# 123456jack/decision-making-and-path-planning

Measured on NVIDIA B200. Metric: trajectories_scored_per_s, higher is better.
Workload: dtype f64

## Files before the change

### decision-making-and-path-planning_b200/csrc/dp_cycle.cu

```cuda
#include <cstdlib>
#include "dp_device.cuh"
#include "dp_fused.cuh"
#include "dp_kernels.h"
#include "dp_group.cuh"

namespace {

struct Beh { int behavior, target, light; bool lanechg, obsavoid; int dlg; };

struct Slice { int base, stride, P; double d; };

__device__ __forceinline__ void put_slot(dp_search_slot* slot, const SearchRes& r, int evaluated, int lane) {
    if (slot && lane == 0) {
        slot->dis_lat = r.dis_lat; slot->dis_lng = r.dis_lng; slot->ob_index = (int16_t)r.ob;
        slot->pathid = (uint16_t)r.pathid; slot->evaluated = (uint8_t)evaluated; slot->found = r.found ? 1 : 0;
        slot->pad[0] = slot->pad[1] = 0;
    }
}

__device__ __forceinline__ void lane_slices(const DevMap& m, int gl, int id, int id_more, Slice& fwd, Slice& rear, int& ub) {
    const int off = m.lane_pt_off[gl], n = m.lane_pt_off[gl + 1] - off;
    const int a = min(n, id + id_more), b = min(n, id + 120 + id_more);
    fwd.base = off + a; fwd.stride = 1; fwd.P = max(0, b - a); fwd.d = 0.0;
    const int lo = max(0, id + id_more - 40);
// ... 32 lines not shown
                sm.scr[j] = m.lenp[off + i0 + j];
            }
            const unsigned bad = __ballot_sync(DP_FULL, !ok);
            if (bad) { first_bad = j0 + __ffs(bad) - 1; break; }
        }
        const int cn = min(cnt, first_bad);
        __syncwarp();
        dp_pad_scr(sm, cn, lane);
        __syncwarp();
        const SeqHit hq = dp_seq_first(sm, cn, sum, 0.0, thr);
        if (hq.k >= 0) return true;
        sum = hq.acc;
        if (first_bad < cnt) break;
    }
    return sum > thr;
}

static __device__ __noinline__ int aim_walk_lane(const DevMap& m, WarpSmem& sm, int gl_walk, int from, int to_excl, float faraim, int lane) {
    if (from >= to_excl) return -2;
    const int off = m.lane_pt_off[gl_walk], n = m.lane_pt_off[gl_walk + 1] - off;
    if (from < 0) return -3;
    if (to_excl > n - 1) { to_excl = n - 1; if (from >= to_excl) return -3; }
    double sum = 0.0;
    for (int i0 = from; i0 < to_excl; i0 += DP_SCR) {
        const int cnt = min(DP_SCR, to_excl - i0);
        __syncwarp();
        for (int j = lane; j < cnt; j += 32) sm.scr[j] = m.lenp[off + i0 + j];
        dp_pad_scr(sm, cnt, lane);
        __syncwarp();
        const SeqHit hq = dp_seq_first(sm, cnt, sum, 4.0, (double)faraim);
        if (hq.k >= 0) return i0 + hq.k;
        sum = hq.acc;
    }
    return -1;
}

__device__ __forceinline__ Src junction_src(const DevMap& m, int base0, int n0, int base1, int n1) {
    Src s = dp_src_run(m.xy + base0, 1, n0);
    s.p1 = m.xy + base1; s.n1 = n1;
    return s;
}

__device__ __forceinline__ void junction_recipe(const DevMap& m, const dp_scene_hdr& h, int& base0, int& n0, int& base1, int& n1) {
    const int gc = (h.conn >= 0 && h.conn < m.n_conn) ? m.conn[h.conn].lane : -1;
    const int coff = gc >= 0 ? m.lane_pt_off[gc] : 0, n_inter = gc >= 0 ? m.lane_pt_off[gc + 1] - coff : 0;
    const int gj = m.road_lane_base[h.road_num - 1] + h.lane_num - 1;
    const int off = m.lane_pt_off[gj], n = m.lane_pt_off[gj + 1] - off;
    if (h.pos == 1) {
        const int idj = (int)(uint16_t)h.id[h.lane_num - 1];
        base0 = off + idj; n0 = max(0, n - idj);
        base1 = coff; n1 = n_inter;
    } else {
        const int idj = (int)(uint16_t)h.id[h.last_lanenum - 1];
        base0 = coff + idj; n0 = max(0, n_inter - idj);
        base1 = off; n1 = min(60, n);
    }
}

static __device__ __noinline__ SearchRes dp_search_cold(const Src s, double mx, double my, const double* ox, const double* oy, int N,
                                                        const LaneMap lm, double lo, double hi, WarpSmem& sm, int lane, float hb = 0.f,
                                                        float dmax = 0.f) {
    return dp_search(s, mx, my, ox, oy, N, lm, lo, hi, sm, lane, hb, dmax);
}

__device__ __forceinline__ void dp_publish(unsigned* flag, unsigned epoch, int lane) {
    __syncwarp();
    if (lane == 0) asm volatile("st.release.gpu.global.u32 [%0], %1;" ::"l"(flag), "r"(epoch) : "memory");
}
__device__ __forceinline__ void dp_await(const unsigned* flag, unsigned epoch) {
    unsigned v = 0;
#pragma unroll 1
    for (int spin = 0; spin < (1 << 22); ++spin) {
        asm volatile("ld.acquire.gpu.global.u32 %0, [%1];" : "=r"(v) : "l"(flag) : "memory");
        if (v == epoch) break;
        __nanosleep(spin < 64 ? 100 : 1000);
    }
    if (v != epoch) __trap();
    __syncwarp();
}
template <class T> __device__ __forceinline__ T dp_l2(const T* p) { return __ldcg(p); }

}

#ifndef DP_PRUNE_REGION
#define DP_PRUNE_REGION 0
#endif
#ifndef DP_PRUNE_LOCAL
#define DP_PRUNE_LOCAL 0
#endif
#ifndef DP_PRUNE_SWEEP
#define DP_PRUNE_SWEEP (WPB == 4)
#endif
#define DP_CARVEOUT 77
#ifndef DP_MIN_BLOCKS_W1
#define DP_MIN_BLOCKS_W1 25
#endif
#define DP_MIN_BLOCKS(WPB) ((WPB) == 1 ? DP_MIN_BLOCKS_W1 : 7)

#ifdef DP_DEBUG_CLOCK
__device__ long long g_dbg_timeline[2 * 65536 * 2 * 8];
__device__ __forceinline__ long long dbg_now() { unsigned long long t; asm volatile("mov.u64 %0, %globaltimer;" : "=l"(t)); return (long long)t; }
#define DBG_MARK(ph, slot) if (lane == 0) g_dbg_timeline[(((size_t)(io.epoch & 1) * 65536 + scene) * 2 + (ph)) * 8 + (slot)] = dbg_now()
#define DBG_END(ph, nt) if (lane == 0) { long long* g = g_dbg_timeline + (((size_t)(io.epoch & 1) * 65536 + scene) * 2 + (ph)) * 8; g[1] = dbg_now(); g[3] = (nt); }
extern "C" int dp_debug_scene_timeline(long long* dst, int n_scenes) {
    (void)n_scenes;
    return (int)cudaMemcpyFromSymbol(dst, g_dbg_timeline, sizeof(g_dbg_timeline));
}
#else
#define DBG_MARK(ph, slot)
#define DBG_END(ph, nt)
#endif

template <int PHASE, int WPB>
__global__ void __launch_bounds__(WPB * 32, DP_MIN_BLOCKS(WPB))
dp_cycle_kernel(DevMap m, dp_params p, int n_scenes, const dp_scene_hdr* __restrict__ hdr, const double* __restrict__ obs_x,
                const double* __restrict__ obs_y, int max_obs, dp_carry* __restrict__ carry, double2* __restrict__ last_path,
                dp_plan_record* __restrict__ rec, dp_trace_record* __restrict__ trace, double* __restrict__ path_xy,
                double* __restrict__ path_ll, DpIo io) {
    __shared__ WarpSmem smem[WPB];
    const int lane = threadIdx.x & 31, wib = threadIdx.x >> 5;
    const int scene = blockIdx.x * WPB + wib;
    if (scene >= n_scenes) return;
#ifdef DP_DEBUG_CLOCK
    if (lane == 0) {
        unsigned sid;
        asm volatile("mov.u32 %0, %smid;" : "=r"(sid));
        long long* g = g_dbg_timeline + (((size_t)(io.epoch & 1) * 65536 + scene) * 2 + (PHASE == 2 ? 1 : 0)) * 8;
        g[0] = dbg_now(); g[2] = sid; g[4] = g[5] = g[6] = 0;
    }
    const long long dbg_t0 = clock64();
    long long dbg_t[8] = {0, 0, 0, 0, 0, 0, 0, 0};
#define DBG_T(i) dbg_t[i] = clock64() - dbg_t0
#else
#define DBG_T(i)
#endif
    WarpSmem& sm = smem[wib];
    if (PHASE == 1 && io.done) asm volatile("griddepcontrol.launch_dependents;" ::: "memory");
    if (PHASE == 2 && io.pdone) asm volatile("griddepcontrol.launch_dependents;" ::: "memory");
    if (PHASE == 1 && io.in_flag) dp_await(io.in_flag, io.epoch);
    if (PHASE == 2 && io.done) dp_await(io.done + scene, io.epoch);
    if (PHASE == 1 && !io.in_flag && !io.hdr_stage && lane < 5) {
        const size_t row = (size_t)scene * max_obs, last = (size_t)(max_obs > 0 ? max_obs - 1 : 0);
        const void* a = lane == 0 ? (const void*)(obs_x + row) : lane == 1 ? (const void*)(obs_x + row + last)
                      : lane == 2 ? (const void*)(obs_y + row) : lane == 3 ? (const void*)(obs_y + row + last) : (const void*)(carry + scene);
        asm volatile("prefetch.global.L2 [%0];" ::"l"(a));
    }
    sm.hdr[lane] = (PHASE == 2 || io.in_flag) ? dp_l2(reinterpret_cast<const uint32_t*>(hdr + scene) + lane)
                                              : reinterpret_cast<const uint32_t*>(hdr + scene)[lane];
    __syncwarp();
    const dp_scene_hdr& h = *reinterpret_cast<const dp_scene_hdr*>(sm.hdr);
    const double* ox = obs_x + (size_t)scene * max_obs;
    const double* oy = obs_y + (size_t)scene * max_obs;
    const int N = min((int)h.n_obs, max_obs);
    if (PHASE != 2 && io.hdr_stage) {
        reinterpret_cast<uint32_t*>(io.hdr_stage + scene)[lane] = sm.hdr[lane];
        for (int k = lane; k < N; k += 32) {
            io.ox_stage[(size_t)scene * max_obs + k] = ox[k];
            io.oy_stage[(size_t)scene * max_obs + k] = oy[k];
        }
    }
    double2* lastp = last_path + (size_t)scene * DP_PATH_POINTS;
    dp_carry* const cg = carry + scene;
    dp_plan_record* const out = rec + scene;
    if (PHASE == 1 && io.prev_epoch) dp_await(io.pdone + scene, io.prev_epoch);
    uint32_t fwd_w = 0;
    if (PHASE != 2 && io.n_fwd) fwd_w = __ldcg(reinterpret_cast<const uint32_t*>(io.fwd_src + scene) + lane);
    const LaneMap lm = dp_lane_map(N, lane);
    const bool lm_act = (lm.nchunk > 1) && (lane < N * lm.nchunk);
    const bool via_l2 = PHASE == 2 || io.in_flag != nullptr;
    const double mx = lm_act ? (via_l2 ? dp_l2(ox + lm.o) : ox[lm.o]) : 0.0, my = lm_act ? (via_l2 ? dp_l2(oy + lm.o) : oy[lm.o]) : 0.0;
    dp_trace_record* tr = trace ? trace + scene : nullptr;
    if (tr && PHASE != 2) {
        uint32_t* w = reinterpret_cast<uint32_t*>(tr);
        for (int i = lane; i < (int)(sizeof(dp_trace_record) / 4); i += 32) w[i] = 0;
        __syncwarp();
    }
    const double Vw = p.vehicle_width;
    const int pos = h.pos;
    int ub = 0, n_traj = 0, pts = 0;
    int rp_base0 = 0, rp_n0 = 0, rp_base1 = 0, rp_n1 = 0;
    int gl = 0, lane_sum = 0;
    const int lane_n = h.lane_num;
    int d_behavior = 1, d_target = 0;
    double v_exp = 10.0;

    if (PHASE == 2) {
        d_behavior = dp_l2(&cg->behavior); d_target = dp_l2(&cg->target_lanenum); v_exp = dp_l2(&cg->velocity_expect);
        n_traj = dp_l2(&out->n_traj);
        if (tr) { ub = dp_l2(&tr->ub_hits); pts = (int)dp_l2(&tr->pts_scored); }
        if (pos == 0) {
            gl = m.road_lane_base[h.road_num - 1] + lane_n - 1;
            lane_sum = m.road_lane_base[h.road_num] - m.road_lane_base[h.road_num - 1];
        } else if (pos == 1 || pos == 2) junction_recipe(m, h, rp_base0, rp_n0, rp_base1, rp_n1);
    } else if (pos == 0) {
        const int road = h.road_num;
        gl = m.road_lane_base[road - 1] + lane_n - 1;
        lane_sum = m.road_lane_base[road] - m.road_lane_base[road - 1];
        const int off = m.lane_pt_off[gl], id_sum = m.lane_pt_off[gl + 1] - off;
        const int id = (int)(uint16_t)h.id[lane_n - 1];
        unsigned navi = 4, navi_t = 0;
        for (int i = 0; i < DP_LANESUM && h.out_lane_no[i] != 0; ++i)
            if (lane_n == h.out_lane_no[i]) { navi = 0; break; }
        int out_min = h.out_lane_no[0], out_max = 1;
        for (int i = 0; i < DP_LANESUM; ++i) if (h.out_lane_no[i] > out_max) out_max = h.out_lane_no[i];
        if (navi == 4) {
            int dirn = 0;
            if (lane_n < out_min) { navi = 2; dirn = 2; }
            else if (lane_n > out_max) { navi = 1; dirn = 1; }
            else navi = 0;
            if (dirn) {
                int times = 5;
                for (int i = 0; i < DP_LANESUM && h.out_lane_no[i] != 0; ++i) {
                    const int t = (dirn == 1) ? lane_n - h.out_lane_no[i] : h.out_lane_no[i] - lane_n;
                    if (t < times) times = t;
                }
                navi_t = (unsigned)(times & 0xff);
            }
        }
        const int idc = min(id, id_sum - 1);
        const int lanechg = m.attr[off + idc];
        const double W = m.width[off + idc] / 100.0;
        Slice F, R, NF, NR;
        NF.base = NR.base = 0; NF.stride = 1; NR.stride = -1; NF.P = NR.P = 0; NF.d = NR.d = 0.0;
        lane_slices(m, gl, id, p.id_more, F, R, ub);
        int side = 0, gn = gl;
        if (lanechg == 1 || lanechg == 3) {
            side = 1;
            if (lane_n > 1) {
                const int idl = (int)(uint16_t)h.id[lane_n - 2];
                const int nl = m.lane_pt_off[gl] - m.lane_pt_off[gl - 1];
                if (idl > 0 && idl < nl) { lane_slices(m, gl - 1, idl, p.id_more, NF, NR, ub); gn = gl - 1; }
            } else { NF = F; NF.d = -1 * W; NR = R; NR.d = -1 * W; }
        } else if (lanechg == 2) {
            side = 2;
            if (lane_n < lane_sum) {
                const int idr = (int)(uint16_t)h.id[lane_n];
                const int nr = m.lane_pt_off[gl + 2] - m.lane_pt_off[gl + 1];
                if (idr > 0 && idr < nr) { lane_slices(m, gl + 1, idr, p.id_more, NF, NR, ub); gn = gl + 1; }
            } else { NF = F; NF.d = W; NR = R; NR.d = W; }
        }
        const int nslot = (side == 2) ? 4 : 2;
        double gF = 0.0, gNF = 0.0, gNR = 0.0;
        double bdF = 0.0;
        {
            const int rb[4] = {F.base, R.base, NF.base, NR.base}, rs[4] = {F.stride, R.stride, NF.stride, NR.stride};
            const int rP[4] = {F.P, R.P, NF.P, NR.P};
            const double rd[4] = {0.0, 0.0, NF.d, NR.d};
            dp_region_stage(m, sm, rb, rs, rP, rd, lane);
            const double nlo = (side == 2) ? -0.5 * W : -0.5 * Vw, nhi = (side == 2) ? 0.5 * Vw : 0.5 * W;
            float hbF, dmF, hbN, dmN;
            dg_bounds(m, gl, 0.0, -0.5 * Vw, 0.5 * Vw, &hbF, &dmF);
            dg_bounds(m, gn, NF.d, nlo, nhi, &hbN, &dmN);
            int qoff = 0;
            bdF = __longlong_as_double(0x7ff0000000000000LL);
#pragma unroll 1
            for (int r = 0; r < 4; ++r) {
                const int Pr = (r == 0) ? F.P : (r == 1) ? R.P : (r == 2) ? NF.P : NR.P;
                if (Pr != 0) {
                    Src sp = dp_src_run(m.xy, 1, Pr);
                    sp.q_off = qoff;
                    const SearchRes sr = dp_search(sp, mx, my, ox, oy, N, lm, r < 2 ? -0.5 * Vw : nlo, r < 2 ? 0.5 * Vw : nhi, sm, lane,
                                                   DP_PRUNE_REGION ? (r < 2 ? hbF : hbN) : 0.f, r < 2 ? dmF : dmN, r == 0 ? &bdF : nullptr);
                    ++n_traj; pts += Pr;
                    put_slot(tr ? &tr->region[r < 2 ? r : nslot + r - 2] : nullptr, sr, 1, lane);
                    if (r == 0) gF = sr.dis_lng; else if (r == 2) gNF = sr.dis_lng; else if (r == 3) gNR = sr.dis_lng;
                }
                qoff += Pr;
            }
        }
        const double gLF = (side == 1) ? gNF : 0.0, gLR = (side == 1) ? gNR : 0.0;
        const double gRF = (side == 2) ? gNF : 0.0, gRR = (side == 2) ? gNR : 0.0;
        if (tr && lane == 0) { tr->width_curlane = W; tr->navi_lanechg = navi; tr->navi_lanechg_times = navi_t; }
        DBG_T(5);
        DBG_MARK(0, 4);

        dp_carry c;
        if (PHASE == 1) {
            const int4* src = reinterpret_cast<const int4*>(cg);
            int4* dst = reinterpret_cast<int4*>(&c);
#pragma unroll
            for (int k = 0; k < (int)(sizeof(dp_carry) / 16); ++k) dst[k] = __ldcg(src + k);
        } else c = *cg;
        Beh cur;
        cur.behavior = c.behavior; cur.target = c.target_lanenum; cur.light = c.light_status;
        cur.lanechg = c.lanechg_status != 0; cur.obsavoid = c.obsavoid_status != 0; cur.dlg = c.behavior_to_dlg;
        const int his_behavior = c.his_behavior, his_target = c.his_target_lanenum, his_light = c.his_light_status;
        int lane_cur = lane_n;
        int z_light = c.light_status;
        int sweep_pick = -1;
        const double period = h.period_ms;
        int K = 0;
        while (K < DP_MAX_SWEEP && (double)K < (W - Vw) / 0.6) ++K;
#define DP_KEEP(reset) do { cur.behavior = 1; cur.target = lane_cur; if (reset) cur.lanechg = false; } while (0)
#define DP_TICK do { c.leftlight_time += period; if (c.leftlight_time > 2000) c.leftlight_time = 2000; } while (0)
        if (lanechg == 0) {
            if (gF < 15) {
                c.no_obsavoid_time = 0;
                c.obsavoid_time++;
                if (c.obsavoid_time > 2) {
                    const int total = 2 * K, shifted = 2 * (K - 1);
                    DBG_MARK(0, 5);
                    if (shifted > 0 && N > 0 && N <= 16) {
                        dp_sweep_stage(m, sm, F.base, F.P, lane);
                        const float hmaxF = m.lane_hmax[gl], hminF = m.lane_hmin[gl], dnF = m.lane_dnmax[gl];
                        unsigned relmask = (N >= 32) ? 0xffffffffu : ((1u << N) - 1u);
                        {
                            const float adm = 0.3f * (float)(K - 1) * 1.0001f;
                            const float hbm = hmaxF + adm * dnF + 1e-4f;
                            const float dlt = (hminF > 1e-6f) ? dnF * (1.0f + 4.0f * adm / hminF) * 1.0001f + 1e-6f : 2.0f;
                            const float dmm = dg_dmax(-0.5 * Vw, 0.5 * Vw, hbm, dlt, hminF - adm * dnF);
                            const bool rel = lane < N && !(sqrt(bdF) - (double)adm > (double)dmm * 1.000001 + 1e-6);
                            relmask &= __ballot_sync(DP_FULL, rel);
                            if (relmask == 0u) relmask = 1u;
                        }
                        const int M = __popc(relmask);
                        const int per = min(8, 32 / M);
                        const int oid = (int)__fns(relmask, 0, lane % M + 1);
                        const double smx = __shfl_sync(DP_FULL, mx, oid), smy = __shfl_sync(DP_FULL, my, oid);
                        for (int u0 = 0; u0 < shifted && (sweep_pick < 0 || tr); u0 += per) {
                            const int cnt = min(per, shifted - u0);
                            const bool none_yet = sweep_pick < 0;
                            int first_g = -1;
                            const int first = dp_sweep_pass(sm, F.P, u0, cnt, K, smx, smy, M, lm, -0.5 * Vw, 0.5 * Vw, 25.0, tr != nullptr, lane,
                                [&](int g, const SearchRes& r, bool before_first) {
                                    if (before_first && r.dis_lng > 25) first_g = g;
                                    if (tr) put_slot(&tr->sweep[(g / K) * DP_MAX_SWEEP + (g % K)], r, (none_yet && before_first) ? 1 : 2, lane);
                                }, DP_PRUNE_SWEEP ? hmaxF : -1.f, hminF, dnF, oid, relmask);
                            if (sweep_pick < 0 && first >= 0) sweep_pick = first_g;
                        }
                    } else {
                        for (int u = 0; u < shifted && (sweep_pick < 0 || tr); ++u) {
                            const int g = dp_sweep_g(u, K);
                            const double cd = dp_sweep_offset(g, K);
                            float hbC, dmC;
                            dg_bounds(m, gl, cd, -0.5 * Vw, 0.5 * Vw, &hbC, &dmC);
                            const SearchRes s = dp_search_cold(slice_src(m, F.base, 1, F.P, cd), mx, my, ox, oy, N, lm, -0.5 * Vw, 0.5 * Vw, sm, lane, hbC, dmC);
                            const bool before = sweep_pick < 0;
                            put_slot(tr ? &tr->sweep[(g / K) * DP_MAX_SWEEP + (g % K)] : nullptr, s, before ? 1 : 2, lane);
                            if (before && s.dis_lng > 25) sweep_pick = g;
                        }
                    }
                    {
                        const int scored = sweep_pick < 0 ? total : sweep_pick + 1;
                        n_traj += scored; pts += scored * F.P;
                        if (tr && total > 0) {
                            __syncwarp();
                            if (lane == 0) {
                                dp_search_slot s0 = tr->region[0];
                                s0.evaluated = 1; tr->sweep[0] = s0;
                                s0.evaluated = (uint8_t)(K < scored ? 1 : 2); tr->sweep[DP_MAX_SWEEP] = s0;
                            }
// ... 741 lines not shown
```

### decision-making-and-path-planning_b200/csrc/dp_device.cuh

```cuda
#pragma once
#include <cuda_runtime.h>
#include <stdint.h>
#include "../../include/dmpp_b200.h"
#include "dp_group.cuh"

#define DP_FULL 0xffffffffu
#define DP_TILE 120
#define DP_SCR 192
#ifndef DP_WARPS_PER_BLOCK
#define DP_WARPS_PER_BLOCK 4
#endif

typedef DgMap DevMap;

struct __align__(16) WarpSmem {
    union {
        struct {
            double2 plan[DP_PATH_POINTS];
            double2 tile[DP_TILE];
        };
        double2 q[DP_PATH_POINTS + DP_TILE];
    };
    double scr[DP_SCR + 8];
    unsigned long long mbar;
    unsigned long long pad_;
    uint32_t hdr[32];
};

struct Src {
    const double2* p0; int stride0; int n0;
    const double2* p1; int n1;
    const double2* nrm0;
    double d;
    int q_off;
};
struct LaneMap { int nchunk, o, c; unsigned magic; };
__device__ __forceinline__ int dp_div_chunks(int x, const LaneMap& lm) { return (int)(((unsigned)x * lm.magic) >> 20); }
struct SearchRes { bool found; double dis_lat, dis_lng; int ob, pathid; };

__device__ __forceinline__ LaneMap dp_lane_map(int N, int lane) {
    LaneMap lm;
    if (N >= 32 || N <= 0) { lm.nchunk = 1; lm.o = lane; lm.c = 0; }
    else { lm.nchunk = 32 / N; lm.c = lane / N; lm.o = lane - lm.c * N; }
    lm.magic = (1u << 20) / (unsigned)lm.nchunk + 1u;
    return lm;
}
__device__ __forceinline__ double dp_sq2(double dx, double dy) { return fma(dx, dx, dy * dy); }
__device__ __forceinline__ double dp_dist_plain(double ax, double ay, double bx, double by) {
    double dx = ax - bx, dy = ay - by;
    return sqrt(dx * dx + dy * dy);
}
__device__ __forceinline__ double2 dp_normal(double2 a, double2 b) {
    double sx = b.x - a.x, sy = b.y - a.y;
    double len = sqrt(dp_sq2(sx, sy));
    if (len > 0) return make_double2(sy / len, -sx / len);
    return make_double2(0.0, 0.0);
}
__device__ __forceinline__ Src dp_src_run(const double2* p, int stride, int n) {
    Src s;
    s.p0 = p; s.stride0 = stride; s.n0 = n; s.p1 = p; s.n1 = 0; s.nrm0 = nullptr; s.d = 0.0; s.q_off = -1;
    return s;
}
__device__ __forceinline__ double2 dp_src_point(const Src& s, int j) {
    if (j >= s.n0) return s.p1[j - s.n0];
    double2 q = s.p0[s.stride0 * j];
    if (s.d != 0.0 && s.n0 >= 2) {
        const int jj = min(j, s.n0 - 2);
        double2 n = (s.stride0 > 0) ? s.nrm0[jj] : s.nrm0[-jj - 1];
        if (s.stride0 < 0) { n.x = -n.x; n.y = -n.y; }
        q.x = fma(s.d, n.x, q.x); q.y = fma(s.d, n.y, q.y);
    }
    return q;
}

__device__ __forceinline__ void dp_pad_scr(WarpSmem& sm, int n, int lane) {
    if (lane < 8) sm.scr[n + lane] = 0.0;
}
__device__ __forceinline__ double dp_seq_sum(const WarpSmem& sm, int n, double acc) {
#pragma unroll 1
    for (int j = 0; j < n; j += 8) {
        const double t0 = sm.scr[j], t1 = sm.scr[j + 1], t2 = sm.scr[j + 2], t3 = sm.scr[j + 3];
        const double t4 = sm.scr[j + 4], t5 = sm.scr[j + 5], t6 = sm.scr[j + 6], t7 = sm.scr[j + 7];
        acc += t0; acc += t1; acc += t2; acc += t3; acc += t4; acc += t5; acc += t6; acc += t7;
    }
    return acc;
}
struct SeqHit { int k; double acc; };
__device__ __forceinline__ SeqHit dp_seq_first(const WarpSmem& sm, int n, double acc, double sub, double thr) {
    SeqHit r;
#pragma unroll 1
    for (int j = 0; j < n; j += 8) {
        const double t0 = sm.scr[j], t1 = sm.scr[j + 1], t2 = sm.scr[j + 2], t3 = sm.scr[j + 3];
        const double t4 = sm.scr[j + 4], t5 = sm.scr[j + 5], t6 = sm.scr[j + 6], t7 = sm.scr[j + 7];
        const double s0 = acc + t0, s1 = s0 + t1, s2 = s1 + t2, s3 = s2 + t3, s4 = s3 + t4, s5 = s4 + t5, s6 = s5 + t6, s7 = s6 + t7;
        if ((s7 - sub) > thr) {
            int k = j + 7;
            if ((s6 - sub) > thr) k = j + 6;
            if ((s5 - sub) > thr) k = j + 5;
            if ((s4 - sub) > thr) k = j + 4;
            if ((s3 - sub) > thr) k = j + 3;
            if ((s2 - sub) > thr) k = j + 2;
            if ((s1 - sub) > thr) k = j + 1;
            if ((s0 - sub) > thr) k = j;
            if (k < n) { r.k = k; r.acc = acc; return r; }
        }
        acc = s7;
    }
    r.k = -1; r.acc = acc;
    return r;
}

__device__ __forceinline__ int dp_nearest_plain(const double2* pts, int n, double x, double y, int lane) {
    const double INF = __longlong_as_double(0x7ff0000000000000LL), TOL = 1.0 + 0x1p-49;
    double be = INF;
    int bi = 0x7fffffff;
    bool amb = false;
    for (int i = lane; i < n; i += 32) {
        const double2 q = pts[i];
        const double dx = x - q.x, dy = y - q.y;
        const double e = dx * dx + dy * dy;
        if (e < be) { amb = amb || (be <= e * TOL); be = e; bi = i; }
    }
    double ge = be;
    int gi = bi;
#pragma unroll
    for (int o = 16; o > 0; o >>= 1) {
        const double oe = __shfl_xor_sync(DP_FULL, ge, o);
        const int oi = __shfl_xor_sync(DP_FULL, gi, o);
        if (oe < ge || (oe == ge && oi < gi)) { ge = oe; gi = oi; }
    }
    amb = amb || (be != ge && be <= ge * TOL);
    if (!__any_sync(DP_FULL, amb)) return (gi != 0x7fffffff && sqrt(ge) < 9999.0) ? gi : 0x7fffffff;
    double md = 9999.0;
    int mi = 0x7fffffff;
    for (int i = lane; i < n; i += 32) {
        const double2 q = pts[i];
        const double dd = dp_dist_plain(x, y, q.x, q.y);
        if (dd < md) { md = dd; mi = i; }
    }
#pragma unroll
    for (int o = 16; o > 0; o >>= 1) {
        const double od = __shfl_xor_sync(DP_FULL, md, o);
        const int oi = __shfl_xor_sync(DP_FULL, mi, o);
        if (od < md || (od == md && oi < mi)) { md = od; mi = oi; }
    }
    return mi;
}

__device__ __forceinline__ uint32_t dp_smem_u32(const void* p) { return (uint32_t)__cvta_generic_to_shared(p); }
__device__ __forceinline__ void dp_bulk_prefetch(void* smem_dst, const void* gmem_src, uint32_t bytes, unsigned long long* mbar, int lane) {
    if (lane == 0) {
        const uint32_t mb = dp_smem_u32(mbar);
        asm volatile("mbarrier.init.shared::cta.b64 [%0], 1;" ::"r"(mb) : "memory");
        asm volatile("fence.proxy.async.shared::cta;" ::: "memory");
        asm volatile("mbarrier.arrive.expect_tx.shared::cta.b64 _, [%0], %1;" ::"r"(mb), "r"(bytes) : "memory");
        asm volatile("cp.async.bulk.shared::cluster.global.mbarrier::complete_tx::bytes [%0], [%1], %2, [%3];"
                     ::"r"(dp_smem_u32(smem_dst)), "l"(gmem_src), "r"(bytes), "r"(mb) : "memory");
    }
    __syncwarp();
}
__device__ __forceinline__ void dp_bulk_wait(unsigned long long* mbar) {
    const uint32_t mb = dp_smem_u32(mbar);
    uint32_t done = 0;
    for (int spin = 0; spin < (1 << 24) && !done; ++spin) {
        asm volatile("{\n .reg .pred p;\n mbarrier.try_wait.parity.shared::cta.b64 p, [%1], 0;\n selp.u32 %0, 1, 0, p;\n}"
                     : "=r"(done) : "r"(mb) : "memory");
    }
    if (!done) __trap();
}

__device__ __forceinline__ SearchRes dp_search(const Src s, double mx, double my, const double* __restrict__ ox,
                                                   const double* __restrict__ oy, int N, const LaneMap lm, double lo, double hi,
                                                   WarpSmem& sm, int lane, const float hb = 0.f, const float dmax = 0.f,
                                                   double* bd_out = nullptr) {
    if (bd_out) *bd_out = __longlong_as_double(0x7ff0000000000000LL);
    SearchRes r;
    r.found = false; r.dis_lat = DP_NOT_FOUND; r.dis_lng = DP_NOT_FOUND; r.ob = -1; r.pathid = 0;
    const int P = s.n0 + s.n1;
    if (P < 2 || N <= 0) return r;
    const int nchunk = lm.nchunk;
    const int CS = (nchunk == 1 || P >= 8192) ? ((nchunk == 1) ? P : (P + nchunk - 1) / nchunk) : dp_div_chunks(P + nchunk - 1, lm);
    const int ngroups = (nchunk == 1) ? (N + 31) >> 5 : 1;
    const bool in_plan = s.q_off >= 0;
    const bool one_tile = in_plan || P <= DP_TILE;
    const double2* pts = &sm.q[in_plan ? s.q_off : DP_PATH_POINTS];
    const double INF = __longlong_as_double(0x7ff0000000000000LL);
    unsigned bestkey = 0xffffffffu;
    double bestd = 0.0;
    for (int g = 0; g < ngroups; ++g) {
        const int o = (nchunk == 1) ? g * 32 + lane : lm.o;
        const bool active = (nchunk == 1) ? (o < N) : (lane < N * nchunk);
        if (nchunk == 1) { mx = active ? __ldcg(ox + o) : 0.0; my = active ? __ldcg(oy + o) : 0.0; }
        const int jlo = lm.c * CS, jhi = active ? min(P, jlo + CS) : 0;
        double b0 = INF, b1 = INF, b2 = INF, b3 = INF;
        int i0 = jlo, i1 = jlo, i2 = jlo, i3 = jlo;
        const int tstep = in_plan ? P : DP_TILE;
        const bool prune = hb > 0.f && one_tile;
        if (prune) {
            if (!in_plan && g == 0) {
                __syncwarp();
                for (int j = lane; j < P; j += 32) sm.tile[j] = dp_src_point(s, j);
                __syncwarp();
            }
            const int len = jhi - jlo;
            if (len > 0) {
                const double2* q = pts + jlo;
                const unsigned long long mk = dg_coarse_f([&](int j) { return q[j]; }, len, mx, my, hb, dmax);
                if (mk) {
                    const DgArg a = dg_refine_f([&](int j) { return q[j]; }, len, mx, my, mk);
                    b0 = a.bd; i0 = jlo + a.bj;
                }
            }
        }
        for (int t0 = 0; t0 < P && !prune; t0 += tstep) {
            const int tn = min(tstep, P - t0);
            if (!in_plan && (g == 0 || !one_tile)) {
                __syncwarp();
                for (int j = lane; j < tn; j += 32) sm.tile[j] = dp_src_point(s, t0 + j);
                __syncwarp();
            }
            int j = max(jlo, t0);
            const int e = min(jhi, t0 + tn);
            const double2* q = pts + (j - t0);
#pragma unroll 2
            for (; j + 4 <= e; j += 4, q += 4) {
                const double2 p0 = q[0], p1 = q[1], p2 = q[2], p3 = q[3];
                const double x0 = mx - p0.x, y0 = my - p0.y, x1 = mx - p1.x, y1 = my - p1.y;
                const double x2 = mx - p2.x, y2 = my - p2.y, x3 = mx - p3.x, y3 = my - p3.y;
                const double d0 = fma(x0, x0, y0 * y0), d1 = fma(x1, x1, y1 * y1);
                const double d2 = fma(x2, x2, y2 * y2), d3 = fma(x3, x3, y3 * y3);
                if (d0 < b0) { b0 = d0; i0 = j; }
                if (d1 < b1) { b1 = d1; i1 = j + 1; }
                if (d2 < b2) { b2 = d2; i2 = j + 2; }
                if (d3 < b3) { b3 = d3; i3 = j + 3; }
            }
            for (; j < e; ++j, ++q) {
                const double2 p0 = q[0];
                const double x0 = mx - p0.x, y0 = my - p0.y;
                const double d0 = fma(x0, x0, y0 * y0);
                if (d0 < b0) { b0 = d0; i0 = j; }
            }
        }
        if (b1 < b0 || (b1 == b0 && i1 < i0)) { b0 = b1; i0 = i1; }
        if (b3 < b2 || (b3 == b2 && i3 < i2)) { b2 = b3; i2 = i3; }
        if (b2 < b0 || (b2 == b0 && i2 < i0)) { b0 = b2; i0 = i2; }
        double bd = b0;
        int bj = i0;
        for (int cc = 1; cc < nchunk; ++cc) {
            const int src = (lm.o + cc * N) & 31;
            const double od = __shfl_sync(DP_FULL, bd, src);
            const int oj = __shfl_sync(DP_FULL, bj, src);
            if (lane < N && od < bd) { bd = od; bj = oj; }
        }
        if (bd_out && nchunk > 1) *bd_out = bd;
        const bool owner = ((nchunk == 1) ? active : (lane < N)) && (!prune || (bd < INF && dg_within_reach(bd, dmax)));
        if (owner) {
            const int k = (bj == P - 1) ? P - 2 : bj;
            const double2 pk = one_tile ? pts[k] : dp_src_point(s, k), pk1 = one_tile ? pts[k + 1] : dp_src_point(s, k + 1);
            const double sx = pk1.x - pk.x, sy = pk1.y - pk.y;
            bool pass = true;
            if (bj == 0) pass = fma(mx - pk.x, sx, (my - pk.y) * sy) >= 0.0;
            else if (bj == P - 1) pass = fma(mx - pk1.x, sx, (my - pk1.y) * sy) <= 0.0;
            const double len = sqrt(dp_sq2(sx, sy));
            double d = 0.0;
            if (len > 0) d = fma(mx - pk.x, sy, -((my - pk.y) * sx)) / len;
            pass = pass && (d >= lo && d <= hi);
            const unsigned key = pass ? (((unsigned)bj << 16) | (unsigned)o) : 0xffffffffu;
            if (key < bestkey) { bestkey = key; bestd = d; }
        }
    }
    const unsigned gmin = __reduce_min_sync(DP_FULL, bestkey);
    if (gmin == 0xffffffffu) return r;
    const int jstar = (int)(gmin >> 16), ostar = (int)(gmin & 0xffffu);
    r.found = true; r.pathid = jstar; r.ob = ostar;
    r.dis_lat = __shfl_sync(DP_FULL, bestd, (nchunk == 1) ? (ostar & 31) : ostar);
    double sum = 0.0;
    for (int t0 = 0; t0 < jstar; t0 += DP_SCR) {
        const int tn = min(DP_SCR, jstar - t0);
        __syncwarp();
        for (int j = lane; j < tn; j += 32) {
            const double2 a = one_tile ? pts[t0 + j] : dp_src_point(s, t0 + j), b = one_tile ? pts[t0 + j + 1] : dp_src_point(s, t0 + j + 1);
            sm.scr[j] = sqrt(dp_sq2(b.x - a.x, b.y - a.y));
        }
        dp_pad_scr(sm, tn, lane);
        __syncwarp();
        sum = dp_seq_sum(sm, tn, sum);
    }
    r.dis_lng = sum;
    return r;
}

static __device__ __noinline__ void dp_sincos_deg(double a, double* c, double* s) {
    const double k = rint(a / 90.0);
    const double r = fma(-90.0, k, a);
    const double x = r * (3.14159265358979323846 / 180.0);
    const double x2 = x * x;
    double ps = -1.0 / 355687428096000.0;
    ps = fma(x2, ps, 1.0 / 1307674368000.0);
    ps = fma(x2, ps, -1.0 / 6227020800.0);
    ps = fma(x2, ps, 1.0 / 39916800.0);
    ps = fma(x2, ps, -1.0 / 362880.0);
    ps = fma(x2, ps, 1.0 / 5040.0);
    ps = fma(x2, ps, -1.0 / 120.0);
    ps = fma(x2, ps, 1.0 / 6.0);
    const double sn = fma(-x * x2, ps, x);
    double pc = 1.0 / 20922789888000.0;
    pc = fma(x2, pc, -1.0 / 87178291200.0);
    pc = fma(x2, pc, 1.0 / 479001600.0);
    pc = fma(x2, pc, -1.0 / 3628800.0);
    pc = fma(x2, pc, 1.0 / 40320.0);
    pc = fma(x2, pc, -1.0 / 720.0);
    pc = fma(x2, pc, 1.0 / 24.0);
    pc = fma(x2, pc, -0.5);
    const double cs = fma(x2, pc, 1.0);
    const long long q = (long long)k;
    const int mq = (int)(((q % 4) + 4) % 4);
    if (mq == 0) { *c = cs; *s = sn; }
    else if (mq == 1) { *c = -sn; *s = cs; }
    else if (mq == 2) { *c = -cs; *s = -sn; }
    else { *c = sn; *s = -cs; }
}

static __device__ __noinline__ double dp_atan(double z) {
    const double PI_2 = 1.57079632679489661923, PI_4 = 0.78539816339744830962;
    const bool neg = z < 0;
    double a = neg ? -z : z;
    const bool inv = a > 1.0;
    if (inv) a = 1.0 / a;
    const bool shift = a > 0.41421356237309503;
    const double w = shift ? (a - 1.0) / (a + 1.0) : a;
    const double w2 = w * w;
    double p = 1.0 / 47.0;
#pragma unroll
    for (int n = 22; n >= 0; --n) {
        const double c = 1.0 / (double)(2 * n + 1);
        p = fma(-w2, p, c);
    }
    double r = w * p;
    if (shift) r = PI_4 + r;
    if (inv) r = PI_2 - r;
    return neg ? -r : r;
}

static __device__ __noinline__ double dp_heading(double ax, double ay, double bx, double by, double eps, double pi) {
    double angle;
    if (fabs(bx - ax) < eps && fabs(by - ay) < eps) angle = 0;
    else if (fabs(bx - ax) < eps) angle = (by > ay) ? pi / 2 : 3 * pi / 2;
    else {
        angle = dp_atan((by - ay) / (bx - ax));
        if (bx < ax) angle = angle + pi;
// ... 90 lines not shown
```

### decision-making-and-path-planning_b200/csrc/dp_fused.cuh

```cuda
#pragma once
#include "dp_device.cuh"

__device__ __forceinline__ void dp_scan(const double2* __restrict__ q, int a, int b, double mx, double my, double& bd, int& bj) {
    const double INF = __longlong_as_double(0x7ff0000000000000LL);
    double b0 = INF, b1 = INF, b2 = INF, b3 = INF;
    int i0 = a, i1 = a, i2 = a, i3 = a;
    int j = a;
    const double2* p = q + a;
    for (; j + 4 <= b; j += 4, p += 4) {
        const double2 p0 = p[0], p1 = p[1], p2 = p[2], p3 = p[3];
        const double x0 = mx - p0.x, y0 = my - p0.y, x1 = mx - p1.x, y1 = my - p1.y;
        const double x2 = mx - p2.x, y2 = my - p2.y, x3 = mx - p3.x, y3 = my - p3.y;
        const double d0 = fma(x0, x0, y0 * y0), d1 = fma(x1, x1, y1 * y1);
        const double d2 = fma(x2, x2, y2 * y2), d3 = fma(x3, x3, y3 * y3);
        if (d0 < b0) { b0 = d0; i0 = j; }
        if (d1 < b1) { b1 = d1; i1 = j + 1; }
        if (d2 < b2) { b2 = d2; i2 = j + 2; }
        if (d3 < b3) { b3 = d3; i3 = j + 3; }
    }
    for (; j < b; ++j, ++p) {
        const double2 p0 = p[0];
        const double x0 = mx - p0.x, y0 = my - p0.y;
        const double d0 = fma(x0, x0, y0 * y0);
        if (d0 < b0) { b0 = d0; i0 = j; }
    }
    if (b1 < b0 || (b1 == b0 && i1 < i0)) { b0 = b1; i0 = i1; }
    if (b3 < b2 || (b3 == b2 && i3 < i2)) { b2 = b3; i2 = i3; }
    if (b2 < b0 || (b2 == b0 && i2 < i0)) { b0 = b2; i0 = i2; }
    bd = b0; bj = i0;
}

__device__ __forceinline__ unsigned dp_owner_key(double2 pk, double2 pk1, int bj, int P, int o, double mx, double my, double lo,
                                                 double hi, double* dout) {
    const double sx = pk1.x - pk.x, sy = pk1.y - pk.y;
    bool pass = true;
    if (bj == 0) pass = fma(mx - pk.x, sx, (my - pk.y) * sy) >= 0.0;
    else if (bj == P - 1) pass = fma(mx - pk1.x, sx, (my - pk1.y) * sy) <= 0.0;
    *dout = 0.0;
    if (!pass) return 0xffffffffu;
    const double cross = fma(mx - pk.x, sy, -((my - pk.y) * sx));
    const double len2 = dp_sq2(sx, sy);
    {
        const float cf = (float)cross, lf = (float)len2;
        const float wm = (float)fmax(fabs(lo), fabs(hi)) * 1.001f + 0.01f;
        if (cf * cf > wm * wm * lf * 1.001f) return 0xffffffffu;
    }
    const double len = sqrt(len2);
    double d = 0.0;
    if (len > 0) d = cross / len;
    *dout = d;
    return (d >= lo && d <= hi) ? (((unsigned)bj << 16) | (unsigned)o) : 0xffffffffu;
}

__device__ __forceinline__ void dp_region_stage(const DevMap& m, WarpSmem& sm, const int (&base)[4], const int (&stride)[4],
                                                const int (&P)[4], const double (&d)[4], int lane) {
    double2* Q = sm.q;
    __syncwarp();
    int S = 0;
#pragma unroll
    for (int r = 0; r < 4; ++r) {
        const int Pr = P[r], bs = base[r], st = stride[r];
        const double dr = d[r];
#pragma unroll
        for (int k = 0; k < ((r & 1) ? 2 : 4); ++k) {
            const int j = lane + 32 * k;
            if (j < Pr) {
                double2 pt = m.xy[bs + st * j];
                if (dr != 0.0 && Pr >= 2) {
                    const int jj = min(j, Pr - 2);
                    double2 n = m.nrm[(st > 0) ? bs + jj : bs - jj - 1];
                    if (st < 0) { n.x = -n.x; n.y = -n.y; }
                    pt.x = fma(dr, n.x, pt.x); pt.y = fma(dr, n.y, pt.y);
                }
                Q[S + j] = pt;
            }
        }
        S += Pr;
    }
    __syncwarp();
}

__device__ __forceinline__ void dp_sweep_stage(const DevMap& m, WarpSmem& sm, int base, int P, int lane) {
    __syncwarp();
    for (int j = lane; j < P; j += 32) {
        sm.q[j] = m.xy[base + j];
        sm.q[128 + j] = (P >= 2) ? m.nrm[base + min(j, P - 2)] : make_double2(0.0, 0.0);
    }
    __syncwarp();
}
__device__ __forceinline__ double2 dp_sweep_point(const WarpSmem& sm, int j, double dc) {
    const double2 p = sm.q[j], n = sm.q[128 + j];
    return make_double2(fma(dc, n.x, p.x), fma(dc, n.y, p.y));
}
__device__ __forceinline__ int dp_sweep_g(int u, int K) { return (u >= K - 1) ? u + 2 : u + 1; }
__device__ __forceinline__ double dp_sweep_offset(int g, int K) { return (g < K) ? -0.3 * g : 0.3 * (g - K); }
template <class Sink>
__device__ __forceinline__ int dp_sweep_pass(WarpSmem& sm, int P, int u0, int cnt, int K, double mx, double my, int N, const LaneMap lm,
                                             double lo, double hi, double clear, bool need_all, int lane, Sink sink,
                                             const float hmax, const float hmin, const float dn, const int oid, const unsigned relmask) {
    const int ci_me = lane / N, o = oid;
    const bool active = ci_me < cnt;
    const int g_me = dp_sweep_g(u0 + ci_me, K);
    const double dc = dp_sweep_offset(g_me, K);
    (void)lm;
    unsigned key = 0xffffffffu;
    double dlat = 0.0;
    if (active && P >= 2) {
        const float ad = (float)fabs(dc) * 1.0001f;
        const float hb = hmax + ad * dn + 1e-4f;
        float delta = dn;
        if (ad > 0.f) delta = (hmin > 1e-6f) ? dn * (1.0f + 4.0f * ad / hmin) * 1.0001f + 1e-6f : 2.0f;
        const float dmax = (hmax < 0.f) ? dg_inff() : dg_dmax(lo, hi, hb, delta, hmin - ad * dn);
        const unsigned long long mk = (hmax < 0.f) ? ~0ull >> (64 - (P + 7) / 8) : dg_coarse_f([&](int j) { return dp_sweep_point(sm, j, dc); }, P, mx, my, hb, dmax);
        DgArg a; a.bd = __longlong_as_double(0x7ff0000000000000LL); a.bj = 0;
        if (mk) a = dg_refine_f([&](int j) { return dp_sweep_point(sm, j, dc); }, P, mx, my, mk);
        const int i0 = a.bj;
        const bool reach = mk && dg_within_reach(a.bd, dmax);
        const int bj = i0, k = (bj == P - 1) ? P - 2 : bj;
        if (reach) key = dp_owner_key(dp_sweep_point(sm, k, dc), dp_sweep_point(sm, k + 1, dc), bj, P, o, mx, my, lo, hi, &dlat);
    }
    int first = -1;
#pragma unroll 1
    for (int ci = 0; ci < cnt; ++ci) {
        if (first >= 0 && !need_all) break;
        const unsigned mine = (ci_me == ci) ? key : 0xffffffffu;
        const unsigned gmin = __reduce_min_sync(DP_FULL, mine);
        SearchRes r;
        r.found = false; r.dis_lat = DP_NOT_FOUND; r.dis_lng = DP_NOT_FOUND; r.ob = -1; r.pathid = 0;
        if (P >= 2 && gmin != 0xffffffffu) {
            const int jstar = (int)(gmin >> 16), ostar = (int)(gmin & 0xffffu);
            r.found = true; r.pathid = jstar; r.ob = ostar;
            r.dis_lat = __shfl_sync(DP_FULL, dlat, ci * N + __popc(relmask & ((1u << ostar) - 1u)));
            const int gc = dp_sweep_g(u0 + ci, K);
            const double dcc = dp_sweep_offset(gc, K);
            int decided = 0;
            if (!need_all && hmax >= 0.f) {
                const float adc = (float)fabs(dcc) * 1.0001f;
                const float tl = hmin - adc * dn, th = hmax + adc * dn;
                if (tl > 0.f && (double)jstar * (double)tl > clear) decided = 1;
                else if ((double)jstar * (double)th <= clear) decided = 2;
            }
            if (decided) r.dis_lng = (decided == 1) ? DP_NOT_FOUND : 0.0;
            else {
                __syncwarp();
                for (int j = lane; j < jstar; j += 32) {
                    const double2 a = dp_sweep_point(sm, j, dcc), b = dp_sweep_point(sm, j + 1, dcc);
                    sm.scr[j] = sqrt(dp_sq2(b.x - a.x, b.y - a.y));
                }
                dp_pad_scr(sm, jstar, lane);
                __syncwarp();
                if (need_all) r.dis_lng = dp_seq_sum(sm, jstar, 0.0);
                else {
                    const SeqHit hq = dp_seq_first(sm, jstar, 0.0, 0.0, clear);
                    r.dis_lng = (hq.k >= 0) ? DP_NOT_FOUND : hq.acc;
                }
            }
        }
        sink(dp_sweep_g(u0 + ci, K), r, first < 0);
        if (first < 0 && r.dis_lng > clear) first = ci;
    }
    return first;
}
// ... 1 lines not shown
```

Baseline: 335.0 million.

## Batch four region searches into one fused warp pass with shared arc-length sum

Replaces the per-region loop of dp_search calls with a single dp_region_search that scans all four regions per obstacle group, merges chunk minima through shared scratch, and computes every region's arc length in one packed window with four lanes summing in parallel. It is meant to remove repeated per-region warp reductions, syncs and sequential arc-length sums. The region pruning bounds (dg_bounds) are dropped, which was already disabled by default. It also adds unroll 2 to the scan loop. Risks include extra shared-memory traffic and more register pressure from the generic lambda sink.

```diff
diff --git a/decision-making-and-path-planning_b200/csrc/dp_cycle.cu b/decision-making-and-path-planning_b200/csrc/dp_cycle.cu
--- a/decision-making-and-path-planning_b200/csrc/dp_cycle.cu
+++ b/decision-making-and-path-planning_b200/csrc/dp_cycle.cu
@@ -138,9 +138,6 @@
 
 }
 
-#ifndef DP_PRUNE_REGION
-#define DP_PRUNE_REGION 0
-#endif
 #ifndef DP_PRUNE_LOCAL
 #define DP_PRUNE_LOCAL 0
 #endif
@@ -279,20 +276,20 @@
         Slice F, R, NF, NR;
         NF.base = NR.base = 0; NF.stride = 1; NR.stride = -1; NF.P = NR.P = 0; NF.d = NR.d = 0.0;
         lane_slices(m, gl, id, p.id_more, F, R, ub);
-        int side = 0, gn = gl;
+        int side = 0;
         if (lanechg == 1 || lanechg == 3) {
             side = 1;
             if (lane_n > 1) {
                 const int idl = (int)(uint16_t)h.id[lane_n - 2];
                 const int nl = m.lane_pt_off[gl] - m.lane_pt_off[gl - 1];
-                if (idl > 0 && idl < nl) { lane_slices(m, gl - 1, idl, p.id_more, NF, NR, ub); gn = gl - 1; }
+                if (idl > 0 && idl < nl) lane_slices(m, gl - 1, idl, p.id_more, NF, NR, ub);
             } else { NF = F; NF.d = -1 * W; NR = R; NR.d = -1 * W; }
         } else if (lanechg == 2) {
             side = 2;
             if (lane_n < lane_sum) {
                 const int idr = (int)(uint16_t)h.id[lane_n];
                 const int nr = m.lane_pt_off[gl + 2] - m.lane_pt_off[gl + 1];
-                if (idr > 0 && idr < nr) { lane_slices(m, gl + 1, idr, p.id_more, NF, NR, ub); gn = gl + 1; }
+                if (idr > 0 && idr < nr) lane_slices(m, gl + 1, idr, p.id_more, NF, NR, ub);
             } else { NF = F; NF.d = W; NR = R; NR.d = W; }
         }
         const int nslot = (side == 2) ? 4 : 2;
@@ -303,26 +300,12 @@
             const int rP[4] = {F.P, R.P, NF.P, NR.P};
             const double rd[4] = {0.0, 0.0, NF.d, NR.d};
             dp_region_stage(m, sm, rb, rs, rP, rd, lane);
-            const double nlo = (side == 2) ? -0.5 * W : -0.5 * Vw, nhi = (side == 2) ? 0.5 * Vw : 0.5 * W;
-            float hbF, dmF, hbN, dmN;
-            dg_bounds(m, gl, 0.0, -0.5 * Vw, 0.5 * Vw, &hbF, &dmF);
-            dg_bounds(m, gn, NF.d, nlo, nhi, &hbN, &dmN);
-            int qoff = 0;
-            bdF = __longlong_as_double(0x7ff0000000000000LL);
-#pragma unroll 1
-            for (int r = 0; r < 4; ++r) {
-                const int Pr = (r == 0) ? F.P : (r == 1) ? R.P : (r == 2) ? NF.P : NR.P;
-                if (Pr != 0) {
-                    Src sp = dp_src_run(m.xy, 1, Pr);
-                    sp.q_off = qoff;
-                    const SearchRes sr = dp_search(sp, mx, my, ox, oy, N, lm, r < 2 ? -0.5 * Vw : nlo, r < 2 ? 0.5 * Vw : nhi, sm, lane,
-                                                   DP_PRUNE_REGION ? (r < 2 ? hbF : hbN) : 0.f, r < 2 ? dmF : dmN, r == 0 ? &bdF : nullptr);
-                    ++n_traj; pts += Pr;
-                    put_slot(tr ? &tr->region[r < 2 ? r : nslot + r - 2] : nullptr, sr, 1, lane);
-                    if (r == 0) gF = sr.dis_lng; else if (r == 2) gNF = sr.dis_lng; else if (r == 3) gNR = sr.dis_lng;
-                }
-                qoff += Pr;
-            }
+            const double rlo[2] = {-0.5 * Vw, (side == 2) ? -0.5 * W : -0.5 * Vw}, rhi[2] = {0.5 * Vw, (side == 2) ? 0.5 * Vw : 0.5 * W};
+            n_traj += (F.P != 0) + (R.P != 0) + (NF.P != 0) + (NR.P != 0); pts += F.P + R.P + NF.P + NR.P;
+            dp_region_search(sm, rP, rlo, rhi, mx, my, ox, oy, N, lm, lane, bdF, [&](int r, const SearchRes& sr) {
+                put_slot(tr ? &tr->region[r < 2 ? r : nslot + r - 2] : nullptr, sr, 1, lane);
+                if (r == 0) gF = sr.dis_lng; else if (r == 2) gNF = sr.dis_lng; else if (r == 3) gNR = sr.dis_lng;
+            });
         }
         const double gLF = (side == 1) ? gNF : 0.0, gLR = (side == 1) ? gNR : 0.0;
         const double gRF = (side == 2) ? gNF : 0.0, gRR = (side == 2) ? gNR : 0.0;
diff --git a/decision-making-and-path-planning_b200/csrc/dp_device.cuh b/decision-making-and-path-planning_b200/csrc/dp_device.cuh
--- a/decision-making-and-path-planning_b200/csrc/dp_device.cuh
+++ b/decision-making-and-path-planning_b200/csrc/dp_device.cuh
@@ -76,9 +76,9 @@
 __device__ __forceinline__ void dp_pad_scr(WarpSmem& sm, int n, int lane) {
     if (lane < 8) sm.scr[n + lane] = 0.0;
 }
-__device__ __forceinline__ double dp_seq_sum(const WarpSmem& sm, int n, double acc) {
+__device__ __forceinline__ double dp_seq_sum(const WarpSmem& sm, int n, double acc, int base = 0) {
 #pragma unroll 1
-    for (int j = 0; j < n; j += 8) {
+    for (int j = base; j < base + n; j += 8) {
         const double t0 = sm.scr[j], t1 = sm.scr[j + 1], t2 = sm.scr[j + 2], t3 = sm.scr[j + 3];
         const double t4 = sm.scr[j + 4], t5 = sm.scr[j + 5], t6 = sm.scr[j + 6], t7 = sm.scr[j + 7];
         acc += t0; acc += t1; acc += t2; acc += t3; acc += t4; acc += t5; acc += t6; acc += t7;
@@ -169,11 +169,22 @@
     if (!done) __trap();
 }
 
+__device__ __forceinline__ unsigned dp_corridor_key(double2 pk, double2 pk1, int bj, int P, int o, double mx, double my, double lo,
+                                                    double hi, double* dout) {
+    const double sx = pk1.x - pk.x, sy = pk1.y - pk.y;
+    bool pass = true;
+    if (bj == 0) pass = fma(mx - pk.x, sx, (my - pk.y) * sy) >= 0.0;
+    else if (bj == P - 1) pass = fma(mx - pk1.x, sx, (my - pk1.y) * sy) <= 0.0;
+    const double len = sqrt(dp_sq2(sx, sy));
+    double d = 0.0;
+    if (len > 0) d = fma(mx - pk.x, sy, -((my - pk.y) * sx)) / len;
+    *dout = d;
+    return (pass && d >= lo && d <= hi) ? (((unsigned)bj << 16) | (unsigned)o) : 0xffffffffu;
+}
+
 __device__ __forceinline__ SearchRes dp_search(const Src s, double mx, double my, const double* __restrict__ ox,
                                                    const double* __restrict__ oy, int N, const LaneMap lm, double lo, double hi,
-                                                   WarpSmem& sm, int lane, const float hb = 0.f, const float dmax = 0.f,
-                                                   double* bd_out = nullptr) {
-    if (bd_out) *bd_out = __longlong_as_double(0x7ff0000000000000LL);
+                                                   WarpSmem& sm, int lane, const float hb = 0.f, const float dmax = 0.f) {
     SearchRes r;
     r.found = false; r.dis_lat = DP_NOT_FOUND; r.dis_lng = DP_NOT_FOUND; r.ob = -1; r.pathid = 0;
     const int P = s.n0 + s.n1;
@@ -252,20 +263,12 @@
             const int oj = __shfl_sync(DP_FULL, bj, src);
             if (lane < N && od < bd) { bd = od; bj = oj; }
         }
-        if (bd_out && nchunk > 1) *bd_out = bd;
         const bool owner = ((nchunk == 1) ? active : (lane < N)) && (!prune || (bd < INF && dg_within_reach(bd, dmax)));
         if (owner) {
             const int k = (bj == P - 1) ? P - 2 : bj;
             const double2 pk = one_tile ? pts[k] : dp_src_point(s, k), pk1 = one_tile ? pts[k + 1] : dp_src_point(s, k + 1);
-            const double sx = pk1.x - pk.x, sy = pk1.y - pk.y;
-            bool pass = true;
-            if (bj == 0) pass = fma(mx - pk.x, sx, (my - pk.y) * sy) >= 0.0;
-            else if (bj == P - 1) pass = fma(mx - pk1.x, sx, (my - pk1.y) * sy) <= 0.0;
-            const double len = sqrt(dp_sq2(sx, sy));
-            double d = 0.0;
-            if (len > 0) d = fma(mx - pk.x, sy, -((my - pk.y) * sx)) / len;
-            pass = pass && (d >= lo && d <= hi);
-            const unsigned key = pass ? (((unsigned)bj << 16) | (unsigned)o) : 0xffffffffu;
+            double d;
+            const unsigned key = dp_corridor_key(pk, pk1, bj, P, o, mx, my, lo, hi, &d);
             if (key < bestkey) { bestkey = key; bestd = d; }
         }
     }
diff --git a/decision-making-and-path-planning_b200/csrc/dp_fused.cuh b/decision-making-and-path-planning_b200/csrc/dp_fused.cuh
--- a/decision-making-and-path-planning_b200/csrc/dp_fused.cuh
+++ b/decision-making-and-path-planning_b200/csrc/dp_fused.cuh
@@ -7,6 +7,7 @@
     int i0 = a, i1 = a, i2 = a, i3 = a;
     int j = a;
     const double2* p = q + a;
+#pragma unroll 2
     for (; j + 4 <= b; j += 4, p += 4) {
         const double2 p0 = p[0], p1 = p[1], p2 = p[2], p3 = p[3];
         const double x0 = mx - p0.x, y0 = my - p0.y, x1 = mx - p1.x, y1 = my - p1.y;
@@ -78,6 +79,120 @@
         S += Pr;
     }
     __syncwarp();
+}
+
+template <class Sink>
+__device__ __forceinline__ void dp_region_search(WarpSmem& sm, const int (&P)[4], const double (&lo)[2], const double (&hi)[2], double mx,
+                                                 double my, const double* __restrict__ ox, const double* __restrict__ oy, int N,
+                                                 const LaneMap lm, int lane, double& bd0, Sink sink) {
+    const double INF = __longlong_as_double(0x7ff0000000000000LL);
+    const int q1 = P[0], q2 = q1 + P[1], q3 = q2 + P[2];
+    double* cbd = sm.scr;
+    int* cbj = reinterpret_cast<int*>(sm.scr + 128);
+    double* lat = sm.scr + DP_SCR;
+    const int nchunk = lm.nchunk;
+    const int nreg = (P[3] >= 2) ? 4 : (P[2] >= 2) ? 3 : (P[1] >= 2) ? 2 : (P[0] >= 2) ? 1 : 0;
+    unsigned k0 = 0xffffffffu, k1 = 0xffffffffu, k2 = 0xffffffffu, k3 = 0xffffffffu;
+    double e0 = 0.0, e1 = 0.0, e2 = 0.0, e3 = 0.0;
+    bd0 = INF;
+#pragma unroll 1
+    for (int g0 = 0; g0 < N; g0 += 32) {
+        const int Ng = min(N - g0, 32);
+        if (nchunk == 1) { mx = lane < Ng ? __ldcg(ox + g0 + lane) : 0.0; my = lane < Ng ? __ldcg(oy + g0 + lane) : 0.0; }
+        __syncwarp();
+#pragma unroll 1
+        for (int r = 0; r < nreg; ++r) {
+            const int Pr = (r == 0) ? P[0] : (r == 1) ? P[1] : (r == 2) ? P[2] : P[3];
+            const int qoff = (r == 0) ? 0 : (r == 1) ? q1 : (r == 2) ? q2 : q3;
+            if (Pr < 2) continue;
+            const int CS = (nchunk == 1) ? Pr : dp_div_chunks(Pr + nchunk - 1, lm);
+            const int jlo = lm.c * CS, jhi = (lane < Ng * nchunk) ? min(Pr, jlo + CS) : 0;
+            double bd;
+            int bj;
+            dp_scan(sm.q + qoff, jlo, jhi, mx, my, bd, bj);
+            cbd[r * 32 + lane] = bd; cbj[r * 32 + lane] = bj;
+        }
+        __syncwarp();
+#pragma unroll 1
+        for (int i = lane; i - lane < nreg * Ng; i += 32) {
+            const int r = (i >= Ng) + (i >= 2 * Ng) + (i >= 3 * Ng), o = i - r * Ng;
+            const double ux = __shfl_sync(DP_FULL, mx, o & 31), uy = __shfl_sync(DP_FULL, my, o & 31);
+            const int Pr = (r == 0) ? P[0] : (r == 1) ? P[1] : (r == 2) ? P[2] : P[3];
+            const int qoff = (r == 0) ? 0 : (r == 1) ? q1 : (r == 2) ? q2 : q3;
+            if (i < nreg * Ng && Pr >= 2) {
+                double bd = cbd[r * 32 + o];
+                int bj = cbj[r * 32 + o];
+                for (int c = 1; c < nchunk; ++c) {
+                    const double od = cbd[r * 32 + c * Ng + o];
+                    const int oj = cbj[r * 32 + c * Ng + o];
+                    if (od < bd) { bd = od; bj = oj; }
+                }
+                if (r == 0 && nchunk > 1) bd0 = bd;
+                const int kk = (bj == Pr - 1) ? Pr - 2 : bj;
+                double d;
+                const unsigned key = dp_corridor_key(sm.q[qoff + kk], sm.q[qoff + kk + 1], bj, Pr, g0 + o, ux, uy,
+                                                     (r < 2) ? lo[0] : lo[1], (r < 2) ? hi[0] : hi[1], &d);
+                if (r == 0 && key < k0) { k0 = key; e0 = d; }
+                if (r == 1 && key < k1) { k1 = key; e1 = d; }
+                if (r == 2 && key < k2) { k2 = key; e2 = d; }
+                if (r == 3 && key < k3) { k3 = key; e3 = d; }
+            }
+        }
+        __syncwarp();
+    }
+    unsigned gmin[4];
+#pragma unroll
+    for (int r = 0; r < 4; ++r) {
+        const unsigned kr = (r == 0) ? k0 : (r == 1) ? k1 : (r == 2) ? k2 : k3;
+        gmin[r] = (r < nreg) ? __reduce_min_sync(DP_FULL, kr) : 0xffffffffu;
+        if (gmin[r] != 0xffffffffu) {
+            const double w = __shfl_sync(DP_FULL, (r == 0) ? e0 : (r == 1) ? e1 : (r == 2) ? e2 : e3,
+                                         __ffs(__ballot_sync(DP_FULL, kr == gmin[r])) - 1);
+            if (lane == 0) lat[r] = w;
+        }
+    }
+    int len[4];
+#pragma unroll
+    for (int r = 0; r < 4; ++r) len[r] = (gmin[r] == 0xffffffffu) ? 0 : (int)(((gmin[r] >> 16) + 7) & ~7u);
+    const int b1 = len[0], b2 = b1 + len[1], b3 = b2 + len[2], T = b3 + len[3];
+    const int my_b = (lane == 1) ? b1 : (lane == 2) ? b2 : (lane == 3) ? b3 : 0;
+    const int my_e = (lane == 0) ? b1 : (lane == 1) ? b2 : (lane == 2) ? b3 : T;
+    double acc = 0.0;
+#pragma unroll 1
+    for (int w = 0; w < T; w += DP_SCR) {
+        const int wn = min(DP_SCR, T - w);
+        __syncwarp();
+        for (int x = lane; x < wn; x += 32) {
+            const int g = w + x;
+            const int r = (g >= b1) + (g >= b2) + (g >= b3);
+            const int j = g - ((r == 0) ? 0 : (r == 1) ? b1 : (r == 2) ? b2 : b3);
+            const int qoff = (r == 0) ? 0 : (r == 1) ? q1 : (r == 2) ? q2 : q3;
+            const unsigned gr = (r == 0) ? gmin[0] : (r == 1) ? gmin[1] : (r == 2) ? gmin[2] : gmin[3];
+            double t = 0.0;
+            if (j < (int)(gr >> 16)) {
+                const double2 a = sm.q[qoff + j], b = sm.q[qoff + j + 1];
+                t = sqrt(dp_sq2(b.x - a.x, b.y - a.y));
+            }
+            sm.scr[x] = t;
+        }
+        __syncwarp();
+        const int a = max(my_b, w), e = min(my_e, w + wn);
+        if (lane < 4 && a < e) acc = dp_seq_sum(sm, e - a, acc, a - w);
+    }
+    __syncwarp();
+#pragma unroll 1
+    for (int r = 0; r < 4; ++r) {
+        const int Pr = (r == 0) ? P[0] : (r == 1) ? P[1] : (r == 2) ? P[2] : P[3];
+        const unsigned gr = (r == 0) ? gmin[0] : (r == 1) ? gmin[1] : (r == 2) ? gmin[2] : gmin[3];
+        SearchRes res;
+        res.found = false; res.dis_lat = DP_NOT_FOUND; res.dis_lng = DP_NOT_FOUND; res.ob = -1; res.pathid = 0;
+        const double lng = __shfl_sync(DP_FULL, acc, r);
+        if (gr != 0xffffffffu) {
+            res.found = true; res.pathid = (int)(gr >> 16); res.ob = (int)(gr & 0xffffu);
+            res.dis_lat = lat[r]; res.dis_lng = lng;
+        }
+        if (Pr != 0) sink(r, res);
+    }
 }
 
 __device__ __forceinline__ void dp_sweep_stage(const DevMap& m, WarpSmem& sm, int base, int P, int lane) {
```

Result: faster. 342.4 million (median of 6 runs) (+2.2%).
